# JuliaDSP/DSP.jl

Hardware: AMD Instinct MI355X
Metric: Gsamples/s filt+welch, 1 Gsample Float32 stream; achieved HBM GB/s vs roofline (higher is better)
Workload: dtype f32; 1 GPU; filt(256 taps, overlap-save nfft 2048) + welch_pgram(nfft 4096, hanning, 50 %) per 2^30-sample Float32 stream; one stream per GPU; RCCL all-reduce of the PSD for N>1; samples_per_gpu=1073741824, engine=fused, collective=none (1 GPU), collective_check=not run (--full checks it)

## Files before the change

### dsp.jl_amd/csrc/fft_lds.h

```cpp
#pragma once

#include <utility>

#ifdef __HIPCC__
#define MDSP_HD __host__ __device__ __forceinline__
#else
#define MDSP_HD inline
#endif
#if defined(__HIP_DEVICE_COMPILE__)
#define MDSP_OPAQUE_INT(x) asm volatile("" : "+v"(x))
#else
#define MDSP_OPAQUE_INT(x) (void)(x)
#endif

namespace mdsp {
namespace fft {

template <typename R> struct cx {
    R x, y;
};

template <typename R> MDSP_HD cx<R> cadd(cx<R> a, cx<R> b) { return {a.x + b.x, a.y + b.y}; }
template <typename R> MDSP_HD cx<R> csub(cx<R> a, cx<R> b) { return {a.x - b.x, a.y - b.y}; }
template <typename R> MDSP_HD cx<R> cmul(cx<R> a, cx<R> b) { return {a.x * b.x - a.y * b.y, a.x * b.y + a.y * b.x}; }
template <typename R> MDSP_HD cx<R> cmulc(cx<R> a, cx<R> b) { return {a.x * b.x + a.y * b.y, a.y * b.x - a.x * b.y}; }
template <int DIR, typename R> MDSP_HD cx<R> twmul(cx<R> a, cx<R> w) { return DIR < 0 ? cmul(a, w) : cmulc(a, w); }
template <int DIR, typename R> MDSP_HD cx<R> mul_mi(cx<R> a) { return DIR < 0 ? cx<R>{a.y, -a.x} : cx<R>{-a.y, a.x}; }

template <int DIR, typename R> MDSP_HD cx<R> add_mi(cx<R> a, cx<R> b) { return cadd(a, mul_mi<DIR>(b)); }
template <int DIR, typename R> MDSP_HD cx<R> sub_mi(cx<R> a, cx<R> b) { return csub(a, mul_mi<DIR>(b)); }
template <typename R> MDSP_HD cx<R> caxpy(R h, cx<R> u, cx<R> e) { return {e.x + h * u.x, e.y + h * u.y}; }
template <typename R> MDSP_HD cx<R> caxmy(R h, cx<R> u, cx<R> e) { return {e.x - h * u.x, e.y - h * u.y}; }
template <typename R> MDSP_HD cx<R> cscale(R h, cx<R> u) { return {h * u.x, h * u.y}; }
template <typename R> MDSP_HD cx<R> lanefma(cx<R> a, cx<R> b, cx<R> c) { return {a.x * b.x + c.x, a.y * b.y + c.y}; }
template <typename R> MDSP_HD cx<R> wmul_hi(cx<R> a, cx<R> w) { return {a.x * w.y, a.y * w.y}; }
template <typename R> MDSP_HD cx<R> wfma_lo(cx<R> a, cx<R> w, cx<R> c) { return {a.x * w.x + c.x, a.y * w.x + c.y}; }
template <typename R> MDSP_HD cx<R> wfms_lo(cx<R> a, cx<R> w, cx<R> c) { return {a.x * w.x - c.x, a.y * w.x - c.y}; }
template <int DIR, typename R> MDSP_HD cx<R> twmul_k(cx<R> a, cx<R> w) { return twmul<DIR>(a, w); }
template <typename R> MDSP_HD cx<R> cscale_k(R h, cx<R> u) { return cscale(h, u); }
template <typename R> MDSP_HD cx<R> caxpy_k(R h, cx<R> u, cx<R> e) { return caxpy(h, u, e); }
template <typename R> MDSP_HD cx<R> caxmy_k(R h, cx<R> u, cx<R> e) { return caxmy(h, u, e); }

#if defined(__HIP_DEVICE_COMPILE__) && !defined(MDSP_NO_PACKED_F32)
typedef float f2v __attribute__((ext_vector_type(2)));
#define MDSP_PK2(NAME, INSN, MODS)                                                                  \
    __device__ __forceinline__ cx<float> NAME(cx<float> a, cx<float> b) {                           \
        f2v d;                                                                                      \
        asm(INSN " %0, %1, %2 " MODS : "=v"(d) : "v"(f2v{a.x, a.y}), "v"(f2v{b.x, b.y}));           \
        return {d.x, d.y};                                                                          \
    }
#define MDSP_PK3(NAME, INSN, MODS)                                                                  \
    __device__ __forceinline__ cx<float> NAME(cx<float> a, cx<float> b, cx<float> c) {              \
        f2v d;                                                                                      \
        asm(INSN " %0, %1, %2, %3 " MODS : "=v"(d) : "v"(f2v{a.x, a.y}), "v"(f2v{b.x, b.y}), "v"(f2v{c.x, c.y})); \
        return {d.x, d.y};                                                                          \
    }
#ifndef MDSP_PK_NATIVE
#define MDSP_PK_NATIVE 0
#endif
#if MDSP_PK_NATIVE
#define MDSP_V(a) (f2v{(a).x, (a).y})
__device__ __forceinline__ cx<float> mdsp_c(f2v d) { return {d.x, d.y}; }
__device__ __forceinline__ cx<float> cadd(cx<float> a, cx<float> b) { return mdsp_c(MDSP_V(a) + MDSP_V(b)); }
__device__ __forceinline__ cx<float> csub(cx<float> a, cx<float> b) { return mdsp_c(MDSP_V(a) - MDSP_V(b)); }
#else
MDSP_PK2(cadd, "v_pk_add_f32", "")
MDSP_PK2(csub, "v_pk_add_f32", "neg_lo:[0,1] neg_hi:[0,1]")
#endif
MDSP_PK2(pk_add_ib, "v_pk_add_f32", "op_sel:[0,1] op_sel_hi:[1,0] neg_lo:[0,1]")
MDSP_PK2(pk_sub_ib, "v_pk_add_f32", "op_sel:[0,1] op_sel_hi:[1,0] neg_hi:[0,1]")
#if MDSP_PK_NATIVE
__device__ __forceinline__ cx<float> pk_mul(cx<float> a, cx<float> b) { return mdsp_c(MDSP_V(a) * MDSP_V(b)); }
__device__ __forceinline__ cx<float> pk_mul_swap(cx<float> a, cx<float> b) { return mdsp_c(f2v{a.y, a.x} * MDSP_V(b)); }
__device__ __forceinline__ cx<float> pk_mul_blo(cx<float> a, cx<float> b) { return mdsp_c(MDSP_V(a) * f2v{b.x, b.x}); }
// ... 128 lines not shown
    b = t;
}

#if defined(__HIP_DEVICE_COMPILE__) && !defined(MDSP_NO_PACKED_F32) && MDSP_PK_FUSED
template <int DIR> __device__ __forceinline__ void bfly4(cx<float>& a0, cx<float>& a1, cx<float>& a2, cx<float>& a3) {
    f2v r0 = {a0.x, a0.y}, r1 = {a1.x, a1.y}, r2 = {a2.x, a2.y}, r3 = {a3.x, a3.y}, t;
    if constexpr (DIR < 0)
        asm("v_pk_add_f32 %4, %0, %2\n\t"
            "v_pk_add_f32 %2, %0, %2 neg_lo:[0,1] neg_hi:[0,1]\n\t"
            "v_pk_add_f32 %0, %1, %3\n\t"
            "v_pk_add_f32 %3, %1, %3 neg_lo:[0,1] neg_hi:[0,1]\n\t"
            "v_pk_add_f32 %1, %4, %0 neg_lo:[0,1] neg_hi:[0,1]\n\t"
            "v_pk_add_f32 %0, %4, %0\n\t"
            "v_pk_add_f32 %4, %2, %3 op_sel:[0,1] op_sel_hi:[1,0] neg_hi:[0,1]\n\t"
            "v_pk_add_f32 %3, %2, %3 op_sel:[0,1] op_sel_hi:[1,0] neg_lo:[0,1]"
            : "+v"(r0), "+v"(r1), "+v"(r2), "+v"(r3), "=&v"(t));
    else
        asm("v_pk_add_f32 %4, %0, %2\n\t"
            "v_pk_add_f32 %2, %0, %2 neg_lo:[0,1] neg_hi:[0,1]\n\t"
            "v_pk_add_f32 %0, %1, %3\n\t"
            "v_pk_add_f32 %3, %1, %3 neg_lo:[0,1] neg_hi:[0,1]\n\t"
            "v_pk_add_f32 %1, %4, %0 neg_lo:[0,1] neg_hi:[0,1]\n\t"
            "v_pk_add_f32 %0, %4, %0\n\t"
            "v_pk_add_f32 %4, %2, %3 op_sel:[0,1] op_sel_hi:[1,0] neg_lo:[0,1]\n\t"
            "v_pk_add_f32 %3, %2, %3 op_sel:[0,1] op_sel_hi:[1,0] neg_hi:[0,1]"
            : "+v"(r0), "+v"(r1), "+v"(r2), "+v"(r3), "=&v"(t));
    a0 = {r0.x, r0.y};
    a1 = {t.x, t.y};
    a2 = {r1.x, r1.y};
    a3 = {r3.x, r3.y};
}
#endif

template <int DIR, typename R> MDSP_HD void bfly4(cx<R>& a0, cx<R>& a1, cx<R>& a2, cx<R>& a3) {
    const cx<R> t0 = cadd(a0, a2), t1 = csub(a0, a2), t2 = cadd(a1, a3), d = csub(a1, a3);
    a0 = cadd(t0, t2);
    a2 = csub(t0, t2);
    a1 = add_mi<DIR>(t1, d);
    a3 = sub_mi<DIR>(t1, d);
}

template <int DIR, typename R> MDSP_HD cx<R> w8_1_unscaled(cx<R> o) { return add_mi<DIR>(o, o); }
template <int DIR, typename R> MDSP_HD cx<R> w8_3_unscaled_neg(cx<R> o) { return sub_mi<DIR>(o, o); }

template <int DIR, typename R> MDSP_HD void bfly8(cx<R> (&v)[8]) {
    constexpr R h = (R)0.70710678118654752440084436210485L;
    bfly4<DIR>(v[0], v[2], v[4], v[6]);
    bfly4<DIR>(v[1], v[3], v[5], v[7]);
    const cx<R> e0 = v[0], e1 = v[2], e2 = v[4], e3 = v[6];
    const cx<R> o0 = v[1], o2 = v[5];
    const cx<R> u1 = w8_1_unscaled<DIR>(v[3]);
    const cx<R> u3 = w8_3_unscaled_neg<DIR>(v[7]);
    v[0] = cadd(e0, o0);
    v[4] = csub(e0, o0);
    v[1] = caxpy_k(h, u1, e1);
    v[5] = caxmy_k(h, u1, e1);
    v[2] = add_mi<DIR>(e2, o2);
    v[6] = sub_mi<DIR>(e2, o2);
    v[3] = caxmy_k(h, u3, e3);
    v[7] = caxpy_k(h, u3, e3);
}

template <int DIR, typename R> MDSP_HD void bfly16_tail(cx<R> (&v)[16]) {
    constexpr R c1 = (R)0.92387953251128675612818318939679L;
    constexpr R s1 = (R)0.38268343236508977172845998403040L;
    constexpr R h = (R)0.70710678118654752440084436210485L;
    const cx<R> w1 = {c1, -s1}, w3 = {s1, -c1}, w9 = {-c1, s1};
    v[1 + 4 * 1] = twmul_k<DIR>(v[1 + 4 * 1], w1);
    v[1 + 4 * 2] = cscale_k(h, w8_1_unscaled<DIR>(v[1 + 4 * 2]));
    v[1 + 4 * 3] = twmul_k<DIR>(v[1 + 4 * 3], w3);
    v[2 + 4 * 1] = cscale_k(h, w8_1_unscaled<DIR>(v[2 + 4 * 1]));
    v[2 + 4 * 2] = mul_mi<DIR>(v[2 + 4 * 2]);
    v[2 + 4 * 3] = cscale_k(-h, w8_3_unscaled_neg<DIR>(v[2 + 4 * 3]));
    v[3 + 4 * 1] = twmul_k<DIR>(v[3 + 4 * 1], w3);
    v[3 + 4 * 2] = cscale_k(-h, w8_3_unscaled_neg<DIR>(v[3 + 4 * 2]));
    v[3 + 4 * 3] = twmul_k<DIR>(v[3 + 4 * 3], w9);
#pragma unroll
    for (int q = 0; q < 4; ++q) bfly4<DIR>(v[4 * q + 0], v[4 * q + 1], v[4 * q + 2], v[4 * q + 3]);
    cx<R> t;
#define MDSP_SWAP(a, b) \
    t = v[a];           \
    v[a] = v[b];        \
    v[b] = t;
    MDSP_SWAP(1, 4) MDSP_SWAP(2, 8) MDSP_SWAP(3, 12) MDSP_SWAP(6, 9) MDSP_SWAP(7, 13) MDSP_SWAP(11, 14)
#undef MDSP_SWAP
}

template <int DIR, typename R> MDSP_HD void bfly16(cx<R> (&v)[16]) {
#pragma unroll
    for (int m = 0; m < 4; ++m) bfly4<DIR>(v[m], v[m + 4], v[m + 8], v[m + 12]);
    bfly16_tail<DIR>(v);
}

template <int DIR, typename R> MDSP_HD void bfly16_win(const cx<R> (&q)[8], const cx<R> (&f)[8], const cx<R> (&wp)[8], cx<R> (&v)[16]) {
#pragma unroll
    for (int m = 0; m < 4; ++m) {
        const cx<R> p0 = wmul_hi(f[m], wp[m]), p1 = wmul_hi(f[m + 4], wp[m + 4]);
        const cx<R> t0 = wfma_lo(q[m], wp[m], p0), t1 = wfms_lo(q[m], wp[m], p0);
        const cx<R> t2 = wfma_lo(q[m + 4], wp[m + 4], p1), d = wfms_lo(q[m + 4], wp[m + 4], p1);
        v[m] = cadd(t0, t2);
        v[m + 8] = csub(t0, t2);
        v[m + 4] = add_mi<DIR>(t1, d);
        v[m + 12] = sub_mi<DIR>(t1, d);
    }
    bfly16_tail<DIR>(v);
}

template <int RDX, int DIR, typename R> MDSP_HD void bfly(cx<R> (&v)[RDX]) {
    if constexpr (RDX == 2) bfly2<DIR>(v[0], v[1]);
    else if constexpr (RDX == 4) bfly4<DIR>(v[0], v[1], v[2], v[3]);
    else if constexpr (RDX == 8) bfly8<DIR>(v);
    else bfly16<DIR>(v);
}

template <int DIR, int RDX, typename R> MDSP_HD void twmul_all(cx<R> (&v)[RDX], const cx<R> (&w)[RDX]) {
#if defined(__HIP_DEVICE_COMPILE__) && !defined(MDSP_NO_PACKED_F32) && MDSP_PK_FUSED
    if constexpr (sizeof(R) == 4) {
#pragma unroll
        for (int r = 1; r + 1 < RDX; r += 2) cmul2(v[r], w[r], v[r + 1], w[r + 1], DIR > 0);
        if constexpr (((RDX - 1) & 1) != 0) v[RDX - 1] = twmul<DIR>(v[RDX - 1], w[RDX - 1]);
        return;
    }
#endif
#pragma unroll
    for (int r = 1; r < RDX; ++r) v[r] = twmul<DIR>(v[r], w[r]);
}

template <int N_, int E_> struct Cfg {
    static constexpr int N = N_, E = E_, T = N_ / E_;
    static constexpr int LOGN = ilog2(N_), LOGE = ilog2(E_);
    static_assert((1 << LOGN) == N_ && (1 << LOGE) == E_, "power of two sizes only");
    static_assert(E_ >= 2 && E_ <= 64 && N_ >= E_, "unsupported elements-per-thread");
    static constexpr int LOGR = LOGE < 4 ? LOGE : 4;
    static constexpr int P = (LOGN + LOGR - 1) / LOGR;
    static constexpr int logradix(int p) { return LOGN / P + (p < LOGN % P ? 1 : 0); }
    static constexpr int radix(int p) { return 1 << logradix(p); }
    static constexpr int ns(int p) { return p == 0 ? 1 : ns(p - 1) * radix(p - 1); }
    static constexpr int ntw(int p) { return p == 0 ? 0 : E - E / radix(p); }
    static constexpr int twoff(int p) { return p == 0 ? 0 : twoff(p - 1) + ntw(p - 1); }
    static constexpr int NTW = twoff(P - 1) + ntw(P - 1);
    static constexpr int ldstw(int p) { return p == 0 ? 0 : (radix(p) - 1) * ns(p); }
    static constexpr int ldsoff(int p) { return p <= 1 ? 0 : ldsoff(p - 1) + ldstw(p - 1); }
    static constexpr int NTWLDS = P <= 1 ? 1 : ldsoff(P - 1) + ldstw(P - 1);
};

enum { TW_GLOBAL = 0, TW_REG = 1, TW_LDS = 2, TW_HYB = 3 };
constexpr int HYB_NS_MAX = 16;
template <typename C, int TWMODE, int PASS> constexpr bool tw_pass_in_lds() {
    return TWMODE == TW_LDS || (TWMODE == TW_HYB && PASS >= 1 && C::ns(PASS) <= HYB_NS_MAX);
}
template <typename C, int TWMODE, int PASS> constexpr bool tw_pass_in_regs() {
    return TWMODE == TW_REG || (TWMODE == TW_HYB && !(PASS >= 1 && C::ns(PASS) <= HYB_NS_MAX));
}
template <typename C, int TWMODE, int PASS = 1> constexpr int tw_lds_entries() {
    if constexpr (PASS >= C::P) return 1;
    else if constexpr (tw_pass_in_lds<C, TWMODE, PASS>()) {
        constexpr int here = C::ldsoff(PASS) + C::ldstw(PASS), rest = tw_lds_entries<C, TWMODE, PASS + 1>();
        return here > rest ? here : rest;
    } else return tw_lds_entries<C, TWMODE, PASS + 1>();
// ... 10 lines not shown
        }
        fill_lds_twiddles<C, R, PASS + 1, TWMODE>(twl, t, table);
    }
}

template <int PADSHIFT> MDSP_HD int lds_pad(int i) {
    if constexpr (PADSHIFT >= 31) return i;
    else return i + (i >> PADSHIFT);
}
template <int N, int PADSHIFT> constexpr int lds_elems() { return PADSHIFT >= 31 ? N : N + (N >> PADSHIFT); }
template <int PADSHIFT> constexpr int lds_padc(int c) { return PADSHIFT >= 31 ? c : c + (c >> PADSHIFT); }

template <typename C, int PASS> MDSP_HD int tw_index(int t, int b, int r) {
    constexpr int Ns = C::ns(PASS), Rdx = C::radix(PASS);
    const int j = t + C::T * b;
    const int k = j & (Ns - 1);
    return (r * k * (C::N / (Ns * Rdx))) & (C::N - 1);
}

template <typename C, typename R, int PASS = 1, int TWMODE = TW_REG>
MDSP_HD void load_twiddles(cx<R> (&tw)[C::NTW > 0 ? C::NTW : 1], int t, const cx<R>* table) {
    if constexpr (PASS < C::P) {
        if constexpr (tw_pass_in_regs<C, TWMODE, PASS>()) {
            constexpr int Rdx = C::radix(PASS), NB = C::E / Rdx;
#pragma unroll
            for (int b = 0; b < NB; ++b)
#pragma unroll
                for (int r = 1; r < Rdx; ++r) tw[C::twoff(PASS) + b * (Rdx - 1) + (r - 1)] = table[tw_index<C, PASS>(t, b, r)];
        }
        load_twiddles<C, R, PASS + 1, TWMODE>(tw, t, table);
    }
}

template <typename C, int DIR, int PASS, int TWMODE, int PADSHIFT, typename R>
MDSP_HD void pass_compute(cx<R> (&x)[C::E], int t, const cx<R> (&tw)[C::NTW > 0 ? C::NTW : 1], const cx<R>* table, cx<R>* lds) {
    constexpr int Rdx = C::radix(PASS), NB = C::E / Rdx, Ns = C::ns(PASS);
    constexpr bool LAST = PASS == C::P - 1;
#pragma unroll
    for (int b = 0; b < NB; ++b) {
        cx<R> v[Rdx];
#pragma unroll
        for (int r = 0; r < Rdx; ++r) v[r] = x[b + r * NB];
        if constexpr (PASS > 0) {
            [[maybe_unused]] int kt = (Ns > C::T) ? t : (t & (Ns - 1));
            constexpr bool IN_LDS = tw_pass_in_lds<C, TWMODE, PASS>(), IN_REGS = tw_pass_in_regs<C, TWMODE, PASS>();
            if constexpr (IN_LDS) MDSP_OPAQUE_INT(kt);
            cx<R> wv[Rdx];
#pragma unroll
            for (int r = 1; r < Rdx; ++r) {
                if constexpr (IN_REGS) wv[r] = tw[C::twoff(PASS) + b * (Rdx - 1) + (r - 1)];
                else if constexpr (IN_LDS) {
                    const int KB = (C::T * b) & (Ns - 1);
                    wv[r] = table[kt + (C::ldsoff(PASS) + (r - 1) * Ns + KB)];
                } else wv[r] = table[tw_index<C, PASS>(t, b, r)];
            }
            twmul_all<DIR, Rdx>(v, wv);
        }
        bfly<Rdx, DIR>(v);
        if constexpr (LAST) {
#pragma unroll
            for (int r = 0; r < Rdx; ++r) x[b + r * NB] = v[r];
        } else {
            const int j = t + C::T * b;
            const int base = lds_pad<PADSHIFT>((j / Ns) * (Ns * Rdx) + (j & (Ns - 1)));
#pragma unroll
            for (int r = 0; r < Rdx; ++r) lds[base + lds_padc<PADSHIFT>(r * Ns)] = v[r];
        }
    }
}

template <typename C, int PADSHIFT, typename R> MDSP_HD void pass0_scatter(const cx<R> (&v)[16], int t, cx<R>* lds) {
    const int base = lds_pad<PADSHIFT>(t * 16);
#pragma unroll
    for (int r = 0; r < 16; ++r) lds[base + lds_padc<PADSHIFT>(r)] = v[r];
}
template <typename C, int PADSHIFT, typename R>
MDSP_HD void pass0_windowed(const cx<R> (&q)[8], const cx<R> (&f)[8], const cx<R> (&wp)[8], int t, cx<R>* lds) {
    static_assert(C::E == 16 && C::radix(0) == 16 && C::P > 1, "E = 16 geometries with a radix-16 first pass");
    cx<R> v[16];
    bfly16_win<-1>(q, f, wp, v);
    pass0_scatter<C, PADSHIFT>(v, t, lds);
}

template <typename C, int PADSHIFT, typename R> MDSP_HD void pass_reload(cx<R> (&x)[C::E], int t, const cx<R>* lds) {
    if constexpr (PADSHIFT >= 31 || C::T % (1 << (PADSHIFT >= 31 ? 0 : PADSHIFT)) == 0) {
        const int base = lds_pad<PADSHIFT>(t);
#pragma unroll
        for (int e = 0; e < C::E; ++e) x[e] = lds[base + lds_padc<PADSHIFT>(C::T * e)];
    } else {
#pragma unroll
        for (int e = 0; e < C::E; ++e) x[e] = lds[lds_pad<PADSHIFT>(t + C::T * e)];
    }
}


template <typename R> MDSP_HD void bfly3f(cx<R>& a0, cx<R>& a1, cx<R>& a2) {
    constexpr R s = (R)0.86602540378443864676372317075294L;
    const cx<R> t1 = cadd(a1, a2), d = csub(a1, a2);
    const cx<R> t2 = caxmy_k((R)0.5, t1, a0);
    const cx<R> t3 = cscale_k(s, d);
    a0 = cadd(a0, t1);
    a1 = add_mi<-1>(t2, t3);
    a2 = sub_mi<-1>(t2, t3);
}
template <typename R> MDSP_HD void bfly5f(cx<R> (&v)[5]) {
    constexpr R c1 = (R)0.30901699437494742410229341718282L, c2 = (R)-0.80901699437494742410229341718282L;
    constexpr R s1 = (R)0.95105651629515357211643933337938L, s2 = (R)0.58778525229247312916870595463907L;
    const cx<R> t1 = cadd(v[1], v[4]), t2 = cadd(v[2], v[3]), t3 = csub(v[1], v[4]), t4 = csub(v[2], v[3]);
    const cx<R> m1 = caxpy_k(c2, t2, caxpy_k(c1, t1, v[0]));
    const cx<R> m2 = caxpy_k(c1, t2, caxpy_k(c2, t1, v[0]));
    const cx<R> n1 = caxpy_k(s2, t4, cscale_k(s1, t3));
    const cx<R> n2 = caxmy_k(s1, t4, cscale_k(s2, t3));
    v[0] = cadd(v[0], cadd(t1, t2));
// ... 196 lines not shown
```

### dsp.jl_amd/csrc/fft_wg.h

```cpp
#pragma once

#include <hip/hip_runtime.h>

#include "fft_lds.h"

#ifndef MDSP_FFT_SETPRIO
#define MDSP_FFT_SETPRIO 0
#endif

namespace mdsp {
namespace fft {

template <int T> __device__ __forceinline__ void wg_sync() {
    if constexpr (T <= 64) __builtin_amdgcn_wave_barrier();
    else __syncthreads();
}

template <typename C, int PADSHIFT, int NBUF> constexpr int wg_lds_elems() { return NBUF * lds_elems<C::N, PADSHIFT>(); }

template <typename C, int DIR, int TWMODE, int PADSHIFT, int NBUF, int XBASE, int PASS = 0, typename R>
__device__ __forceinline__ void wg_fft(cx<R> (&v)[C::E], int t, const cx<R> (&tw)[C::NTW > 0 ? C::NTW : 1], const cx<R>* table, cx<R>* lds) {
    constexpr int BUF = (XBASE + PASS) % NBUF;
    cx<R>* region = lds + BUF * lds_elems<C::N, PADSHIFT>();
    pass_compute<C, DIR, PASS, TWMODE, PADSHIFT>(v, t, tw, table, region);
    if constexpr (PASS < C::P - 1) {
#if MDSP_FFT_SETPRIO
        __builtin_amdgcn_s_setprio(1);
#endif
        wg_sync<C::T>();
        pass_reload<C, PADSHIFT>(v, t, region);
        if constexpr (NBUF == 1) wg_sync<C::T>();
#if MDSP_FFT_SETPRIO
        __builtin_amdgcn_s_setprio(0);
#endif
        wg_fft<C, DIR, TWMODE, PADSHIFT, NBUF, XBASE, PASS + 1>(v, t, tw, table, lds);
    }
}

template <typename C, int TWMODE, typename R>
__device__ __forceinline__ const cx<R>* wg_twiddle_setup(cx<R> (&tw)[C::NTW > 0 ? C::NTW : 1], cx<R>* twl, int t, int slot, const cx<R>* table) {
    if constexpr (TWMODE == TW_REG) {
        load_twiddles<C, R, 1, TW_REG>(tw, t, table);
        return table;
    } else if constexpr (TWMODE == TW_LDS) {
        if (slot == 0) fill_lds_twiddles<C, R>(twl, t, table);
        __syncthreads();
        return twl;
    } else if constexpr (TWMODE == TW_HYB) {
        load_twiddles<C, R, 1, TW_HYB>(tw, t, table);
        if (slot == 0) fill_lds_twiddles<C, R, 1, TW_HYB>(twl, t, table);
        __syncthreads();
        return twl;
    } else {
        return table;
    }
}

template <typename C> constexpr int wg_exchanges() { return C::P - 1; }

}
}
```

### dsp.jl_amd/csrc/ols.hip

```cpp
#include <algorithm>
#include <atomic>
#include <cstdlib>

#ifndef MDSP_FFT_SGPR_CONST
#define MDSP_FFT_SGPR_CONST 0
#endif

#include "common.h"
#include "devio.h"
#include "fft_lds.h"
#include "fft_wg.h"
#include "hostfft.h"
#include "rocfft_wrap.h"
#include "ols_plan.h"

using namespace mdsp;
using mdsp::fft::cx;

namespace {

template <typename T>
__global__ __launch_bounds__(256) void ols_segment_kernel(const T* __restrict__ x, T* __restrict__ td, int64_t nx, int64_t ldx,
                                                          int64_t nblocks, int64_t L, int nb, int nfft, int64_t u0, int64_t nunits) {
    const int64_t u = u0 + blockIdx.x;
// ... 93 lines not shown
    {
        const __amdgpu_buffer_rsrc_t r = io::make_rsrc(xc + start, q.live ? (a.nx - start) * SZ : 0);
        const int lead = __builtin_amdgcn_readfirstlane((int)(start < 0 ? -start : 0));
        io::load_window<TT, E, T>(raw.a, r, lead, t);
    }
    if constexpr (!CPLX) {
        const bool haveB = q.live && (g0 + 1) < a.nblocks;
        const int64_t startB = start + a.L;
        const __amdgpu_buffer_rsrc_t r = io::make_rsrc(xc + startB, haveB ? (a.nx - startB) * SZ : 0);
        const int lead = __builtin_amdgcn_readfirstlane((int)(startB < 0 ? -startB : 0));
        io::load_window<TT, E, T>(raw.b, r, lead, t);
    }
}

template <typename R, int E, int T, bool CPLX>
__device__ __forceinline__ void ols_store(const cx<R> (&v)[E], const OlsFusedArgs& a, OlsPos q, int t) {
    using TT = std::conditional_t<CPLX, cx<R>, R>;
    constexpr int64_t SZ = (int64_t)sizeof(TT);
    const int64_t off0 = (CPLX ? q.p : 2 * q.p) * a.L;
    const int lead = a.nb - 1;
    TT* yc = static_cast<TT*>(a.y) + q.col * a.ldy;
    {
        const __amdgpu_buffer_rsrc_t w = io::make_rsrc(yc + off0 - lead, q.live ? (a.nout - off0 + lead) * SZ : 0);
        if constexpr (CPLX) io::store_window<TT, E, T>([&](int e) { return v[e]; }, w, lead, t);
        else io::store_window<TT, E, T>([&](int e) { return v[e].x; }, w, lead, t);
    }
    if constexpr (!CPLX) {
        const int64_t offB = off0 + a.L;
        const __amdgpu_buffer_rsrc_t w = io::make_rsrc(yc + offB - lead, (q.live && offB < a.nout) ? (a.nout - offB + lead) * SZ : 0);
        io::store_window<TT, E, T>([&](int e) { return v[e].y; }, w, lead, t);
    }
}

template <typename R, int N, int E, int G, int TWMODE, bool CPLX, int NBUF, bool PREFETCH, bool HREG = true, bool ROWS = false>
__global__ __launch_bounds__((N / E) * G, 2) void ols_fused_kernel(OlsFusedArgs a) {
    static_assert(!ROWS || (CPLX && !HREG), "the rows form: complex blocks, one spectrum row per block");
    using C = fft::Cfg<N, E>;
    constexpr int T = C::T, PADSHIFT = 4;
    static_assert(T % 64 == 0, "a transform must own whole wavefronts (uniform descriptors)");
    constexpr int NTWA = C::NTW > 0 ? C::NTW : 1;
    constexpr int REGION = fft::wg_lds_elems<C, PADSHIFT, NBUF>();
    __shared__ __attribute__((aligned(16))) cx<R> lds_all[G * REGION];
    const int t = threadIdx.x % T;
    const int slot = __builtin_amdgcn_readfirstlane((int)(threadIdx.x / T));
    cx<R>* lds = lds_all + slot * REGION;
    const cx<R>* table = static_cast<const cx<R>*>(a.table);

    cx<R> tw[NTWA];
    __shared__ __attribute__((aligned(16))) cx<R> twl[(TWMODE == fft::TW_LDS || TWMODE == fft::TW_HYB) ? fft::tw_lds_entries<C, TWMODE>() : 1];
    const cx<R>* twsrc = fft::wg_twiddle_setup<C, TWMODE>(tw, twl, t, slot, table);
    cx<R> Hr[HREG ? E : 1];
    if constexpr (HREG) {
#pragma unroll
        for (int e = 0; e < E; ++e) Hr[e] = static_cast<const cx<R>*>(a.H)[t + T * e];
    }
    const __amdgpu_buffer_rsrc_t hrsrc = io::make_rsrc(a.H, (int64_t)N * (int64_t)sizeof(cx<R>));

    const int64_t nslots = (int64_t)gridDim.x * G;
    OlsWalk walk{a.u_begin + ((int64_t)blockIdx.x * G + slot) * a.run_len, 0};
    OlsPos cur = ols_pos(a, walk, a.niter > 0);
    OlsRaw<R, E, CPLX> raw;
    if constexpr (PREFETCH) ols_issue_loads<R, E, T, CPLX>(raw, a, cur, t);
    for (int64_t it = 0; it < a.niter; ++it) {
        ols_walk_next(walk, a.run_len, nslots);
        const OlsPos nxt = ols_pos(a, walk, it + 1 < a.niter);
        if constexpr (!PREFETCH) {
            if (!MDSP_ABLATED(a, 1)) {
                if (a.memprio & 1) __builtin_amdgcn_s_setprio(3);
                ols_issue_loads<R, E, T, CPLX>(raw, a, cur, t);
                if (a.memprio & 1) __builtin_amdgcn_s_setprio(0);
            }
        }
        cx<R> v[E];
#pragma unroll
        for (int e = 0; e < E; ++e) {
            if constexpr (CPLX) v[e] = raw.a[e];
            else v[e] = {raw.a[e], raw.b[e]};
        }
        if constexpr (PREFETCH) { if (!MDSP_ABLATED(a, 1)) ols_issue_loads<R, E, T, CPLX>(raw, a, nxt, t); }
        if (!MDSP_ABLATED(a, 2)) {
        fft::wg_fft<C, -1, TWMODE, PADSHIFT, NBUF, 0>(v, t, tw, twsrc, lds);
        if constexpr (HREG) {
#pragma unroll
            for (int e = 0; e < E; ++e) v[e] = fft::cmul(v[e], Hr[e]);
        } else {
            cx<R> hh[E];
            if constexpr (ROWS) {
                const __amdgpu_buffer_rsrc_t hrow = io::make_rsrc(static_cast<const cx<R>*>(a.H) + (cur.p % a.hrows) * N, (int64_t)N * (int64_t)sizeof(cx<R>));
                io::load_window<cx<R>, E, T>(hh, hrow, 0, t);
            } else
            io::load_window<cx<R>, E, T>(hh, hrsrc, 0, t);
#pragma unroll
            for (int e = 0; e < E; ++e) v[e] = fft::cmul(v[e], hh[e]);
        }
        fft::wg_fft<C, +1, TWMODE, PADSHIFT, NBUF, (C::P - 1) % NBUF>(v, t, tw, twsrc, lds);
        if constexpr (ROWS) {
            const cx<R>*t0 = static_cast<const cx<R>*>(a.rt0), *t1 = static_cast<const cx<R>*>(a.rt1);
            const unsigned k1 = (unsigned)(cur.p % a.hrows), mask = (1u << a.rlogS) - 1u;
            const auto root = [&](unsigned m) { return fft::cmul(t0[m & mask], t1[m >> a.rlogS]); };
            const cx<R> w0 = root(k1 * (unsigned)t);
#pragma unroll
            for (int e = 0; e < E; ++e) {
                const cx<R> w = fft::cmul(w0, root(k1 * (unsigned)(T * e)));
                v[e] = fft::cmul(v[e], cx<R>{w.x, -w.y});
            }
        }
        }
        if (!MDSP_ABLATED(a, 4)) {
            if (a.memprio & 2) __builtin_amdgcn_s_setprio(3);
            ols_store<R, E, T, CPLX>(v, a, cur, t);
            if (a.memprio & 2) __builtin_amdgcn_s_setprio(0);
        }
        cur = nxt;
    }
}

struct UpolsArgs {
    const void* x;
    void* y;
    const void* table;
    const void* Hp;
    int64_t nx, nout, ldx, ldy;
    int64_t nblocks;
    int64_t g_begin;
    int64_t x_lo;
    int64_t run_len;
    int ablate;
    int memprio;
// ... 365 lines not shown
        return true;
    }
    for (int64_t n = 4096; n <= nmax; n *= 2) {
        const int64_t parts = cdiv(nb, n / 2);
        if (parts <= 4) {
            *exec_nfft = n;
            *partitions = (int)std::max<int64_t>(2, parts);
            return true;
        }
    }
    return false;
}

template <typename R> int upload_spectrum(mdsp_ols_plan_s* pl, const std::vector<zd>& Hfull, bool half) {
    const int64_t n = half ? pl->nfft / 2 + 1 : pl->nfft;
    std::vector<cx<R>> h((size_t)n);
    for (int64_t k = 0; k < n; ++k) h[(size_t)k] = {(R)Hfull[(size_t)k].real(), (R)Hfull[(size_t)k].imag()};
    MDSP_TRY(pl->H.reserve(sizeof(cx<R>) * (size_t)n));
    MDSP_HIP(hipMemcpy(pl->H.p, h.data(), sizeof(cx<R>) * (size_t)n, hipMemcpyHostToDevice));
    return MDSP_OK;
}

template <typename R> int upload_table(DevBuf& buf, int64_t n) {
    std::vector<cx<R>> w((size_t)n);
    for (int64_t k = 0; k < n; ++k) {
        const zd r = unit_root(k, n, -1);
        w[(size_t)k] = {(R)r.real(), (R)r.imag()};
    }
    MDSP_TRY(buf.reserve(sizeof(cx<R>) * (size_t)n));
    MDSP_HIP(hipMemcpy(buf.p, w.data(), sizeof(cx<R>) * (size_t)n, hipMemcpyHostToDevice));
    return MDSP_OK;
}

template <typename R, int N, int E, int G, int TWMODE, bool CPLX, int NBUF, bool PREFETCH, bool HREG = true, bool ROWS = false>
int launch_fused_geo(const OlsFusedArgs& a, hipStream_t s) {
    auto kern = ols_fused_kernel<R, N, E, G, TWMODE, CPLX, NBUF, PREFETCH, HREG, ROWS>;
    constexpr int threads = (N / E) * G;
    int per_cu = 0;
    MDSP_HIP(hipOccupancyMaxActiveBlocksPerMultiprocessor(&per_cu, kern, threads, 0));
    if (per_cu < 1) per_cu = 1;
    if (tunables().wg_per_cu > 0) per_cu = tunables().wg_per_cu;
    const int64_t todo = a.nunits - a.u_begin;
    const int64_t want = cdiv(todo, G);
    const int grid = (int)std::max<int64_t>(1, std::min<int64_t>(want, (int64_t)device_cu_count() * per_cu));
    OlsFusedArgs b = a;
    const int64_t runs = tunables().runs_per_slot;
    const int64_t nslots = (int64_t)grid * G;
    b.run_len = std::max<int64_t>(1, cdiv(todo, nslots * runs));
    b.niter = cdiv(cdiv(todo, b.run_len), nslots) * b.run_len;
    hipLaunchKernelGGL(kern, dim3(grid), dim3(threads), 0, s, b);
    MDSP_LAUNCH_CHECK();
    return MDSP_OK;
}

int ols_rows_impl(int dbl, void* work, int64_t rows, int hrows, const void* Hrows, const void* table, const void* rt0, const void* rt1, int rlogS, hipStream_t st) {
    OlsFusedArgs a{};
    const int64_t S = dbl ? 4096 : 8192;
    a.x = work;
    a.y = work;
    a.table = table;
    a.H = Hrows;
    a.nx = a.nout = a.ldx = a.ldy = rows * S;
    a.L = S;
    a.nb = 1;
    a.nblocks = a.units_per_col = a.nunits = rows;
    a.u_begin = 0;
    a.memprio = tunables().ols_prio;
    a.hrows = hrows;
    a.rt0 = rt0;
    a.rt1 = rt1;
    a.rlogS = rlogS;
    if (dbl) return launch_fused_geo<double, 4096, 8, 1, 1, true, 2, false, false, true>(a, st);
    return launch_fused_geo<float, 8192, 16, 1, 1, true, 1, false, false, true>(a, st);
}

template <typename R, int N, bool CPLX> int launch_fused_n(const OlsFusedArgs& a, hipStream_t s) {
    constexpr bool DBL = sizeof(R) == 8;
    constexpr int EMAX = (!DBL && N >= 1024) ? 16 : 8;
    constexpr int E = (N / 64 < EMAX) ? N / 64 : EMAX;
    constexpr int T = N / E;
    constexpr int G = slots_per_workgroup(T);
    constexpr int NBUF = (T <= 64 || E == 16) ? 1 : 2;
#ifndef MDSP_TW_F64
#define MDSP_TW_F64 1
#endif
    constexpr int TWREG = DBL ? MDSP_TW_F64 : 1;
    if constexpr (N == 2048 && !CPLX && !DBL) return launch_fused_geo<R, N, 16, 1, 1, CPLX, 1, false>(a, s);
    if (tunables().ols_prefetch == 1) return launch_fused_geo<R, N, E, G, TWREG, CPLX, NBUF, true>(a, s);
    return launch_fused_geo<R, N, E, G, TWREG, CPLX, NBUF, false>(a, s);
}

template <typename R, bool CPLX> int launch_fused(int64_t nfft, const OlsFusedArgs& a, hipStream_t s) {
    switch (nfft) {
        case 256: return launch_fused_n<R, 256, CPLX>(a, s);
        case 512: return launch_fused_n<R, 512, CPLX>(a, s);
        case 1024: return launch_fused_n<R, 1024, CPLX>(a, s);
        case 2048: return launch_fused_n<R, 2048, CPLX>(a, s);
        case 4096: return launch_fused_n<R, 4096, CPLX>(a, s);
        case 8192:
            if constexpr (sizeof(R) == 4) return launch_fused_n<R, 8192, CPLX>(a, s);
        default: break;
    }
    MDSP_FAIL(MDSP_ERR_UNSUPPORTED, "fused overlap-save does not support nfft=%lld", (long long)nfft);
}

struct UpolsRange {
    int64_t g0, g1, x_lo;
};
template <typename R, int N, int E, int P, bool CPLX, int MINW, bool XDMA, int NLDS = 0, int FORM = 1, bool H0REG = false>
int launch_upols_k(const mdsp_ols_plan_s* pl, const void* x, int64_t nx, int64_t ncols, int64_t ldx, void* y, int64_t nout, int64_t ldy, UpolsRange rg, hipStream_t s) {
    constexpr bool DBL = sizeof(R) == 8;
    constexpr int TW = DBL ? 1 : fft::TW_HYB;
    void (*kern)(UpolsArgs) = nullptr;
    if constexpr (FORM == 2) kern = upols2_fused_kernel<R, N, E, P, TW, 4, CPLX, MINW, NLDS, H0REG>;
    else kern = upols_fused_kernel<R, N, E, P, TW, 4, CPLX, MINW, XDMA, NLDS>;
    constexpr int threads = N / E, RUNS = CPLX ? 1 : 2;
    UpolsArgs a;
    a.x = x; a.y = y; a.table = pl->table.p; a.Hp = pl->H.p;
    a.nx = nx; a.nout = nout; a.ldx = ldx; a.ldy = ldy;
    a.nblocks = rg.g1;
    a.g_begin = rg.g0;
    a.x_lo = rg.x_lo;
// ... 422 lines not shown
```

Baseline: 366.8 Gsamples/s.

## Fold twiddle multiplies into radix-16/8 butterflies and fuse spectrum multiply into inverse FFT

Adds folded butterfly variants that merge each twiddle multiply into the first butterfly stage with FMA (including packed-f32 inline-asm versions). For the real nfft=2048 overlap-save path it also folds the filter spectrum multiply into the first radix-16 pass of the inverse FFT, and uses folded twiddle passes for later stages. The aim is fewer VALU instructions per FFT in a kernel that may be compute-bound. In exchange it adds a large amount of hand-written asm with intricate modifier encodings, which risks numerical or sign errors and could raise register pressure.

```diff
diff --git a/dsp.jl_amd/csrc/fft_lds.h b/dsp.jl_amd/csrc/fft_lds.h
--- a/dsp.jl_amd/csrc/fft_lds.h
+++ b/dsp.jl_amd/csrc/fft_lds.h
@@ -40,6 +40,22 @@
 template <typename R> MDSP_HD cx<R> cscale_k(R h, cx<R> u) { return cscale(h, u); }
 template <typename R> MDSP_HD cx<R> caxpy_k(R h, cx<R> u, cx<R> e) { return caxpy(h, u, e); }
 template <typename R> MDSP_HD cx<R> caxmy_k(R h, cx<R> u, cx<R> e) { return caxmy(h, u, e); }
+
+MDSP_HD float fma1(float a, float b, float c) { return __builtin_fmaf(a, b, c); }
+MDSP_HD double fma1(double a, double b, double c) { return __builtin_fma(a, b, c); }
+template <typename R> struct cx2 {
+    cx<R> plus, minus;
+};
+template <int DIR, typename R> MDSP_HD cx2<R> fold(cx<R> a, cx<R> b, cx<R> w) {
+    const R wy = DIR < 0 ? w.y : -w.y;
+    const cx<R> t = {fma1(b.y, -wy, a.x), fma1(b.y, w.x, a.y)};
+    const cx<R> p = {fma1(b.x, w.x, t.x), fma1(b.x, wy, t.y)};
+    return {p, {fma1(a.x, (R)2, -p.x), fma1(a.y, (R)2, -p.y)}};
+}
+template <int DIR, typename R> MDSP_HD cx2<R> fold_mi(cx<R> a, cx<R> b) { return {add_mi<DIR>(a, b), sub_mi<DIR>(a, b)}; }
+template <typename R> MDSP_HD cx2<R> fold_re(cx<R> a, R h, cx<R> u) {
+    return {{fma1(u.x, h, a.x), fma1(u.y, h, a.y)}, {fma1(-u.x, h, a.x), fma1(-u.y, h, a.y)}};
+}
 
 #if defined(__HIP_DEVICE_COMPILE__) && !defined(MDSP_NO_PACKED_F32)
 typedef float f2v __attribute__((ext_vector_type(2)));
@@ -234,6 +250,90 @@
 }
 #endif
 
+#if defined(__HIP_DEVICE_COMPILE__) && !defined(MDSP_NO_PACKED_F32) && MDSP_PK_FUSED
+#define MDSP_M_SUB " neg_lo:[0,1] neg_hi:[0,1]"
+#define MDSP_M_ADD_IB " op_sel:[0,1] op_sel_hi:[1,0] neg_lo:[0,1]"
+#define MDSP_M_SUB_IB " op_sel:[0,1] op_sel_hi:[1,0] neg_hi:[0,1]"
+#define MDSP_M_YY " op_sel:[1,1] op_sel_hi:[1,0]"
+#define MDSP_M_FIN_F " op_sel_hi:[0,1,1] neg_lo:[0,0,1]"
+#define MDSP_M_FIN_I " op_sel_hi:[0,1,1] neg_hi:[1,0,0]"
+#define MDSP_M_FA_F " op_sel:[1,1,0] op_sel_hi:[1,0,1] neg_lo:[0,1,0]"
+#define MDSP_M_FA_I " op_sel:[1,1,0] op_sel_hi:[1,0,1]"
+#define MDSP_M_FB_F " op_sel_hi:[0,1,1]"
+#define MDSP_M_FB_I " op_sel_hi:[0,1,1] neg_hi:[0,1,0]"
+#define MDSP_M_F2 " op_sel_hi:[1,0,1] neg_lo:[0,0,1] neg_hi:[0,0,1]"
+#define MDSP_M_NEGA " neg_lo:[1,0,0] neg_hi:[1,0,0]"
+#define MDSP_BFLY4_TW(FA, FB, X1, X3)                                                                                         \
+    asm("v_pk_fma_f32 %4, %2, %6, %0" FA "\n\tv_pk_fma_f32 %5, %3, %7, %1" FA "\n\t"                                            \
+        "v_pk_fma_f32 %4, %2, %6, %4" FB "\n\tv_pk_fma_f32 %5, %3, %7, %5" FB "\n\t"                      \
+        "v_pk_fma_f32 %2, %0, 2.0, %4" MDSP_M_F2 "\n\tv_pk_fma_f32 %3, %1, 2.0, %5" MDSP_M_F2 "\n\t"        \
+        "v_pk_add_f32 %0, %4, %5\n\tv_pk_add_f32 %1, %4, %5" MDSP_M_SUB "\n\t"                                                  \
+        "v_pk_add_f32 %4, %2, %3" X1 "\n\tv_pk_add_f32 %3, %2, %3" X3                                                           \
+        : "+v"(r0), "+v"(r1), "+v"(r2), "+v"(r3), "=&v"(t), "=&v"(u) : "v"(f2v{w2.x, w2.y}), "v"(f2v{w3.x, w3.y}))
+template <int DIR, int WDIR> __device__ __forceinline__ void bfly4_tw(cx<float>& a0, cx<float>& a1, cx<float>& a2, cx<float>& a3, cx<float> w2, cx<float> w3) {
+    f2v r0 = {a0.x, a0.y}, r1 = {a1.x, a1.y}, r2 = {a2.x, a2.y}, r3 = {a3.x, a3.y}, t, u;
+    if constexpr (DIR < 0 && WDIR < 0) MDSP_BFLY4_TW(MDSP_M_FA_F, MDSP_M_FB_F, MDSP_M_SUB_IB, MDSP_M_ADD_IB);
+    else if constexpr (DIR < 0) MDSP_BFLY4_TW(MDSP_M_FA_I, MDSP_M_FB_I, MDSP_M_SUB_IB, MDSP_M_ADD_IB);
+    else if constexpr (WDIR < 0) MDSP_BFLY4_TW(MDSP_M_FA_F, MDSP_M_FB_F, MDSP_M_ADD_IB, MDSP_M_SUB_IB);
+    else MDSP_BFLY4_TW(MDSP_M_FA_I, MDSP_M_FB_I, MDSP_M_ADD_IB, MDSP_M_SUB_IB);
+    a0 = {r0.x, r0.y};
+    a1 = {t.x, t.y};
+    a2 = {r1.x, r1.y};
+    a3 = {r3.x, r3.y};
+}
+#undef MDSP_BFLY4_TW
+#define MDSP_BFLY4_W16_13(FIN, UMOD, T0NEG, T1NEG, FA, FB, X1, X3)                                                              \
+    asm("v_pk_mul_f32 %4, %1, %6" MDSP_M_YY "\n\tv_pk_add_f32 %5, %2, %2" UMOD "\n\t"                                             \
+        "v_pk_fma_f32 %4, %1, %6, %4" FIN "\n\t"                                                              \
+        "v_pk_fma_f32 %1, %5, %7, %0" T0NEG "\n\tv_pk_fma_f32 %2, %5, %7, %0" T1NEG "\n\t"                  \
+        "v_pk_fma_f32 %5, %3, %8, %4" FA "\n\tv_pk_fma_f32 %5, %3, %8, %5" FB "\n\t"                                 \
+        "v_pk_fma_f32 %3, %4, 2.0, %5" MDSP_M_F2 "\n\t"                                                              \
+        "v_pk_add_f32 %0, %1, %5\n\tv_pk_add_f32 %4, %1, %5" MDSP_M_SUB "\n\t"                                                    \
+        "v_pk_add_f32 %1, %2, %3" X1 "\n\tv_pk_add_f32 %3, %2, %3" X3                                                             \
+        : "+v"(r0), "+v"(r1), "+v"(r2), "+v"(r3), "=&v"(t), "=&v"(u) : "v"(f2v{wa.x, wa.y}), "v"(f2v{h, h}), "v"(f2v{wb.x, wb.y}))
+#define MDSP_BFLY4_W16_2(MI_ADD, MI_SUB)                                                                                         \
+    asm("v_pk_add_f32 %4, %1, %1" MI_ADD "\n\tv_pk_add_f32 %5, %3, %3" MI_SUB "\n\t"                                              \
+        "v_pk_mul_f32 %4, %4, %6\n\t"                                                                            \
+        "v_pk_add_f32 %1, %0, %2" MI_ADD "\n\tv_pk_add_f32 %2, %0, %2" MI_SUB "\n\t"                        \
+        "v_pk_fma_f32 %0, %5, %6, %4" MDSP_M_NEGA "\n\tv_pk_fma_f32 %3, %5, %6, %4\n\t"                      \
+        "v_pk_add_f32 %5, %1, %0\n\tv_pk_add_f32 %4, %1, %0" MDSP_M_SUB "\n\t"                                                    \
+        "v_pk_add_f32 %1, %2, %3" MI_ADD "\n\tv_pk_add_f32 %3, %2, %3" MI_SUB                                                     \
+        : "+v"(r0), "+v"(r1), "+v"(r2), "+v"(r3), "=&v"(t), "=&v"(u) : "v"(f2v{h, h}))
+template <int DIR, int Q> __device__ __forceinline__ void bfly4_w16(cx<float>& a0, cx<float>& a1, cx<float>& a2, cx<float>& a3) {
+    constexpr float c1 = 0.92387953251128675612818318939679f, s1 = 0.38268343236508977172845998403040f, h = 0.70710678118654752440084436210485f;
+    constexpr cx<float> wa = Q == 1 ? cx<float>{c1, -s1} : cx<float>{s1, -c1}, wb = Q == 1 ? cx<float>{s1, -c1} : cx<float>{-c1, s1};
+    f2v r0 = {a0.x, a0.y}, r1 = {a1.x, a1.y}, r2 = {a2.x, a2.y}, r3 = {a3.x, a3.y}, t, u;
+    if constexpr (Q == 2) {
+        if constexpr (DIR < 0) MDSP_BFLY4_W16_2(MDSP_M_SUB_IB, MDSP_M_ADD_IB);
+        else MDSP_BFLY4_W16_2(MDSP_M_ADD_IB, MDSP_M_SUB_IB);
+        a0 = {u.x, u.y};
+    } else {
+        if constexpr (Q == 1 && DIR < 0) MDSP_BFLY4_W16_13(MDSP_M_FIN_F, MDSP_M_SUB_IB, "", MDSP_M_NEGA, MDSP_M_FA_F, MDSP_M_FB_F, MDSP_M_SUB_IB, MDSP_M_ADD_IB);
+        else if constexpr (Q == 1) MDSP_BFLY4_W16_13(MDSP_M_FIN_I, MDSP_M_ADD_IB, "", MDSP_M_NEGA, MDSP_M_FA_I, MDSP_M_FB_I, MDSP_M_ADD_IB, MDSP_M_SUB_IB);
+        else if constexpr (DIR < 0) MDSP_BFLY4_W16_13(MDSP_M_FIN_F, MDSP_M_ADD_IB, MDSP_M_NEGA, "", MDSP_M_FA_F, MDSP_M_FB_F, MDSP_M_SUB_IB, MDSP_M_ADD_IB);
+        else MDSP_BFLY4_W16_13(MDSP_M_FIN_I, MDSP_M_SUB_IB, MDSP_M_NEGA, "", MDSP_M_FA_I, MDSP_M_FB_I, MDSP_M_ADD_IB, MDSP_M_SUB_IB);
+        a0 = {r0.x, r0.y};
+    }
+    a1 = {r1.x, r1.y};
+    a2 = {t.x, t.y};
+    a3 = {r3.x, r3.y};
+}
+#undef MDSP_BFLY4_W16_13
+#undef MDSP_BFLY4_W16_2
+#undef MDSP_M_SUB
+#undef MDSP_M_ADD_IB
+#undef MDSP_M_SUB_IB
+#undef MDSP_M_YY
+#undef MDSP_M_FIN_F
+#undef MDSP_M_FIN_I
+#undef MDSP_M_FA_F
+#undef MDSP_M_FA_I
+#undef MDSP_M_FB_F
+#undef MDSP_M_FB_I
+#undef MDSP_M_F2
+#undef MDSP_M_NEGA
+#endif
+
 template <int DIR, typename R> MDSP_HD void bfly4(cx<R>& a0, cx<R>& a1, cx<R>& a2, cx<R>& a3) {
     const cx<R> t0 = cadd(a0, a2), t1 = csub(a0, a2), t2 = cadd(a1, a3), d = csub(a1, a3);
     a0 = cadd(t0, t2);
@@ -245,10 +345,8 @@
 template <int DIR, typename R> MDSP_HD cx<R> w8_1_unscaled(cx<R> o) { return add_mi<DIR>(o, o); }
 template <int DIR, typename R> MDSP_HD cx<R> w8_3_unscaled_neg(cx<R> o) { return sub_mi<DIR>(o, o); }
 
-template <int DIR, typename R> MDSP_HD void bfly8(cx<R> (&v)[8]) {
+template <int DIR, typename R> MDSP_HD void bfly8_tail(cx<R> (&v)[8]) {
     constexpr R h = (R)0.70710678118654752440084436210485L;
-    bfly4<DIR>(v[0], v[2], v[4], v[6]);
-    bfly4<DIR>(v[1], v[3], v[5], v[7]);
     const cx<R> e0 = v[0], e1 = v[2], e2 = v[4], e3 = v[6];
     const cx<R> o0 = v[1], o2 = v[5];
     const cx<R> u1 = w8_1_unscaled<DIR>(v[3]);
@@ -262,8 +360,49 @@
     v[3] = caxmy_k(h, u3, e3);
     v[7] = caxpy_k(h, u3, e3);
 }
-
-template <int DIR, typename R> MDSP_HD void bfly16_tail(cx<R> (&v)[16]) {
+template <int DIR, typename R> MDSP_HD void bfly8(cx<R> (&v)[8]) {
+    bfly4<DIR>(v[0], v[2], v[4], v[6]);
+    bfly4<DIR>(v[1], v[3], v[5], v[7]);
+    bfly8_tail<DIR>(v);
+}
+
+template <int DIR, int WDIR, typename R> MDSP_HD void bfly4_tw(cx<R>& a0, cx<R>& a1, cx<R>& a2, cx<R>& a3, cx<R> w2, cx<R> w3) {
+    const cx2<R> e = fold<WDIR>(a0, a2, w2), o = fold<WDIR>(a1, a3, w3);
+    a0 = cadd(e.plus, o.plus);
+    a2 = csub(e.plus, o.plus);
+    a1 = add_mi<DIR>(e.minus, o.minus);
+    a3 = sub_mi<DIR>(e.minus, o.minus);
+}
+template <int DIR, int Q, typename R> MDSP_HD void bfly4_w16(cx<R>& a0, cx<R>& a1, cx<R>& a2, cx<R>& a3) {
+    constexpr R c1 = (R)0.92387953251128675612818318939679L, s1 = (R)0.38268343236508977172845998403040L, h = (R)0.70710678118654752440084436210485L;
+    const cx<R> w1 = {c1, -s1}, w3 = {s1, -c1}, w9 = {-c1, s1};
+    cx2<R> e, o;
+    if constexpr (Q == 1) {
+        const cx<R> p = twmul_k<DIR>(a1, w1);
+        e = fold_re(a0, h, w8_1_unscaled<DIR>(a2));
+        o = fold<DIR>(p, a3, w3);
+    } else if constexpr (Q == 2) {
+        const cx<R> p = cscale_k(h, w8_1_unscaled<DIR>(a1));
+        e = fold_mi<DIR>(a0, a2);
+        o = fold_re(p, -h, w8_3_unscaled_neg<DIR>(a3));
+    } else {
+        const cx<R> p = twmul_k<DIR>(a1, w3);
+        e = fold_re(a0, -h, w8_3_unscaled_neg<DIR>(a2));
+        o = fold<DIR>(p, a3, w9);
+    }
+    a0 = cadd(e.plus, o.plus);
+    a2 = csub(e.plus, o.plus);
+    a1 = add_mi<DIR>(e.minus, o.minus);
+    a3 = sub_mi<DIR>(e.minus, o.minus);
+}
+
+template <int DIR, bool FOLD = false, typename R> MDSP_HD void bfly16_tail(cx<R> (&v)[16]) {
+    if constexpr (FOLD) {
+        bfly4<DIR>(v[0], v[1], v[2], v[3]);
+        bfly4_w16<DIR, 1>(v[4], v[5], v[6], v[7]);
+        bfly4_w16<DIR, 2>(v[8], v[9], v[10], v[11]);
+        bfly4_w16<DIR, 3>(v[12], v[13], v[14], v[15]);
+    } else {
     constexpr R c1 = (R)0.92387953251128675612818318939679L;
     constexpr R s1 = (R)0.38268343236508977172845998403040L;
     constexpr R h = (R)0.70710678118654752440084436210485L;
@@ -279,6 +418,7 @@
     v[3 + 4 * 3] = twmul_k<DIR>(v[3 + 4 * 3], w9);
 #pragma unroll
     for (int q = 0; q < 4; ++q) bfly4<DIR>(v[4 * q + 0], v[4 * q + 1], v[4 * q + 2], v[4 * q + 3]);
+    }
     cx<R> t;
 #define MDSP_SWAP(a, b) \
     t = v[a];           \
@@ -288,10 +428,10 @@
 #undef MDSP_SWAP
 }
 
-template <int DIR, typename R> MDSP_HD void bfly16(cx<R> (&v)[16]) {
+template <int DIR, bool FOLD = false, typename R> MDSP_HD void bfly16(cx<R> (&v)[16]) {
 #pragma unroll
     for (int m = 0; m < 4; ++m) bfly4<DIR>(v[m], v[m + 4], v[m + 8], v[m + 12]);
-    bfly16_tail<DIR>(v);
+    bfly16_tail<DIR, FOLD>(v);
 }
 
 template <int DIR, typename R> MDSP_HD void bfly16_win(const cx<R> (&q)[8], const cx<R> (&f)[8], const cx<R> (&wp)[8], cx<R> (&v)[16]) {
@@ -327,6 +467,33 @@
 #pragma unroll
     for (int r = 1; r < RDX; ++r) v[r] = twmul<DIR>(v[r], w[r]);
 }
+
+template <int WDIR, int RDX, bool W0, typename R> MDSP_HD void twmul_first(cx<R> (&v)[RDX], const cx<R> (&w)[RDX]) {
+    constexpr int HALF = RDX / 2, R0 = W0 ? 0 : 1;
+#if defined(__HIP_DEVICE_COMPILE__) && !defined(MDSP_NO_PACKED_F32) && MDSP_PK_FUSED
+    if constexpr (sizeof(R) == 4) {
+#pragma unroll
+        for (int r = R0; r + 1 < HALF; r += 2) cmul2(v[r], w[r], v[r + 1], w[r + 1], WDIR > 0);
+        if constexpr (((HALF - R0) & 1) != 0) v[HALF - 1] = twmul<WDIR>(v[HALF - 1], w[HALF - 1]);
+        return;
+    }
+#endif
+#pragma unroll
+    for (int r = R0; r < HALF; ++r) v[r] = twmul<WDIR>(v[r], w[r]);
+}
+template <int DIR, int WDIR = DIR, bool W0 = false, typename R> MDSP_HD void bfly16_tw(cx<R> (&v)[16], const cx<R> (&w)[16]) {
+    twmul_first<WDIR, 16, W0>(v, w);
+#pragma unroll
+    for (int m = 0; m < 4; ++m) bfly4_tw<DIR, WDIR>(v[m], v[m + 4], v[m + 8], v[m + 12], w[m + 8], w[m + 12]);
+    bfly16_tail<DIR, true>(v);
+}
+template <int DIR, typename R> MDSP_HD void bfly8_tw(cx<R> (&v)[8], const cx<R> (&w)[8]) {
+    twmul_first<DIR, 8, false>(v, w);
+    bfly4_tw<DIR, DIR>(v[0], v[2], v[4], v[6], w[4], w[6]);
+    bfly4_tw<DIR, DIR>(v[1], v[3], v[5], v[7], w[5], w[7]);
+    bfly8_tail<DIR>(v);
+}
+template <int DIR, typename R> MDSP_HD void bfly16_h(cx<R> (&v)[16], const cx<R> (&H)[16]) { bfly16_tw<DIR, -1, true>(v, H); }
 
 template <int N_, int E_> struct Cfg {
     static constexpr int N = N_, E = E_, T = N_ / E_;
@@ -403,10 +570,11 @@
     }
 }
 
-template <typename C, int DIR, int PASS, int TWMODE, int PADSHIFT, typename R>
+template <typename C, int DIR, int PASS, int TWMODE, int PADSHIFT, bool FOLD = false, typename R>
 MDSP_HD void pass_compute(cx<R> (&x)[C::E], int t, const cx<R> (&tw)[C::NTW > 0 ? C::NTW : 1], const cx<R>* table, cx<R>* lds) {
     constexpr int Rdx = C::radix(PASS), NB = C::E / Rdx, Ns = C::ns(PASS);
     constexpr bool LAST = PASS == C::P - 1;
+    constexpr bool FOLDED_TW = FOLD && PASS > 0 && (Rdx == 16 || Rdx == 8);
 #pragma unroll
     for (int b = 0; b < NB; ++b) {
         cx<R> v[Rdx];
@@ -425,9 +593,14 @@
                     wv[r] = table[kt + (C::ldsoff(PASS) + (r - 1) * Ns + KB)];
                 } else wv[r] = table[tw_index<C, PASS>(t, b, r)];
             }
-            twmul_all<DIR, Rdx>(v, wv);
+            if constexpr (FOLDED_TW && Rdx == 16) bfly16_tw<DIR>(v, wv);
+            else if constexpr (FOLDED_TW) bfly8_tw<DIR>(v, wv);
+            else twmul_all<DIR, Rdx>(v, wv);
         }
-        bfly<Rdx, DIR>(v);
+        if constexpr (!FOLDED_TW) {
+            if constexpr (FOLD && Rdx == 16) bfly16<DIR, true>(v);
+            else bfly<Rdx, DIR>(v);
+        }
         if constexpr (LAST) {
 #pragma unroll
             for (int r = 0; r < Rdx; ++r) x[b + r * NB] = v[r];
@@ -450,6 +623,12 @@
     static_assert(C::E == 16 && C::radix(0) == 16 && C::P > 1, "E = 16 geometries with a radix-16 first pass");
     cx<R> v[16];
     bfly16_win<-1>(q, f, wp, v);
+    pass0_scatter<C, PADSHIFT>(v, t, lds);
+}
+
+template <typename C, int DIR, int PADSHIFT, typename R> MDSP_HD void pass0_spectrum(cx<R> (&v)[16], const cx<R> (&H)[16], int t, cx<R>* lds) {
+    static_assert(C::E == 16 && C::radix(0) == 16 && C::P > 1, "E = 16 geometries with a radix-16 first pass");
+    bfly16_h<DIR>(v, H);
     pass0_scatter<C, PADSHIFT>(v, t, lds);
 }
 
diff --git a/dsp.jl_amd/csrc/fft_wg.h b/dsp.jl_amd/csrc/fft_wg.h
--- a/dsp.jl_amd/csrc/fft_wg.h
+++ b/dsp.jl_amd/csrc/fft_wg.h
@@ -18,11 +18,11 @@
 
 template <typename C, int PADSHIFT, int NBUF> constexpr int wg_lds_elems() { return NBUF * lds_elems<C::N, PADSHIFT>(); }
 
-template <typename C, int DIR, int TWMODE, int PADSHIFT, int NBUF, int XBASE, int PASS = 0, typename R>
+template <typename C, int DIR, int TWMODE, int PADSHIFT, int NBUF, int XBASE, int PASS = 0, bool FOLD = false, typename R>
 __device__ __forceinline__ void wg_fft(cx<R> (&v)[C::E], int t, const cx<R> (&tw)[C::NTW > 0 ? C::NTW : 1], const cx<R>* table, cx<R>* lds) {
     constexpr int BUF = (XBASE + PASS) % NBUF;
     cx<R>* region = lds + BUF * lds_elems<C::N, PADSHIFT>();
-    pass_compute<C, DIR, PASS, TWMODE, PADSHIFT>(v, t, tw, table, region);
+    pass_compute<C, DIR, PASS, TWMODE, PADSHIFT, FOLD>(v, t, tw, table, region);
     if constexpr (PASS < C::P - 1) {
 #if MDSP_FFT_SETPRIO
         __builtin_amdgcn_s_setprio(1);
@@ -33,8 +33,17 @@
 #if MDSP_FFT_SETPRIO
         __builtin_amdgcn_s_setprio(0);
 #endif
-        wg_fft<C, DIR, TWMODE, PADSHIFT, NBUF, XBASE, PASS + 1>(v, t, tw, table, lds);
+        wg_fft<C, DIR, TWMODE, PADSHIFT, NBUF, XBASE, PASS + 1, FOLD>(v, t, tw, table, lds);
     }
+}
+
+template <typename C, int DIR, int TWMODE, int PADSHIFT, typename R>
+__device__ __forceinline__ void wg_fft_spectrum(cx<R> (&v)[C::E], const cx<R> (&H)[C::E], int t, const cx<R> (&tw)[C::NTW > 0 ? C::NTW : 1], const cx<R>* table, cx<R>* lds) {
+    pass0_spectrum<C, DIR, PADSHIFT>(v, H, t, lds);
+    wg_sync<C::T>();
+    pass_reload<C, PADSHIFT>(v, t, lds);
+    wg_sync<C::T>();
+    wg_fft<C, DIR, TWMODE, PADSHIFT, 1, 0, 1, true>(v, t, tw, table, lds);
 }
 
 template <typename C, int TWMODE, typename R>
diff --git a/dsp.jl_amd/csrc/ols.hip b/dsp.jl_amd/csrc/ols.hip
--- a/dsp.jl_amd/csrc/ols.hip
+++ b/dsp.jl_amd/csrc/ols.hip
@@ -149,9 +149,10 @@
     }
 }
 
-template <typename R, int N, int E, int G, int TWMODE, bool CPLX, int NBUF, bool PREFETCH, bool HREG = true, bool ROWS = false>
+template <typename R, int N, int E, int G, int TWMODE, bool CPLX, int NBUF, bool PREFETCH, bool HREG = true, bool ROWS = false, bool FOLD = false>
 __global__ __launch_bounds__((N / E) * G, 2) void ols_fused_kernel(OlsFusedArgs a) {
     static_assert(!ROWS || (CPLX && !HREG), "the rows form: complex blocks, one spectrum row per block");
+    static_assert(!FOLD || (HREG && NBUF == 1 && E == 16), "the folded form: spectrum in registers, one LDS buffer");
     using C = fft::Cfg<N, E>;
     constexpr int T = C::T, PADSHIFT = 4;
     static_assert(T % 64 == 0, "a transform must own whole wavefronts (uniform descriptors)");
@@ -196,7 +197,10 @@
         }
         if constexpr (PREFETCH) { if (!MDSP_ABLATED(a, 1)) ols_issue_loads<R, E, T, CPLX>(raw, a, nxt, t); }
         if (!MDSP_ABLATED(a, 2)) {
-        fft::wg_fft<C, -1, TWMODE, PADSHIFT, NBUF, 0>(v, t, tw, twsrc, lds);
+        fft::wg_fft<C, -1, TWMODE, PADSHIFT, NBUF, 0, 0, FOLD>(v, t, tw, twsrc, lds);
+        if constexpr (FOLD) {
+            fft::wg_fft_spectrum<C, +1, TWMODE, PADSHIFT>(v, Hr, t, tw, twsrc, lds);
+        } else {
         if constexpr (HREG) {
 #pragma unroll
             for (int e = 0; e < E; ++e) v[e] = fft::cmul(v[e], Hr[e]);
@@ -211,6 +215,7 @@
             for (int e = 0; e < E; ++e) v[e] = fft::cmul(v[e], hh[e]);
         }
         fft::wg_fft<C, +1, TWMODE, PADSHIFT, NBUF, (C::P - 1) % NBUF>(v, t, tw, twsrc, lds);
+        }
         if constexpr (ROWS) {
             const cx<R>*t0 = static_cast<const cx<R>*>(a.rt0), *t1 = static_cast<const cx<R>*>(a.rt1);
             const unsigned k1 = (unsigned)(cur.p % a.hrows), mask = (1u << a.rlogS) - 1u;
@@ -642,9 +647,9 @@
     return MDSP_OK;
 }
 
-template <typename R, int N, int E, int G, int TWMODE, bool CPLX, int NBUF, bool PREFETCH, bool HREG = true, bool ROWS = false>
+template <typename R, int N, int E, int G, int TWMODE, bool CPLX, int NBUF, bool PREFETCH, bool HREG = true, bool ROWS = false, bool FOLD = false>
 int launch_fused_geo(const OlsFusedArgs& a, hipStream_t s) {
-    auto kern = ols_fused_kernel<R, N, E, G, TWMODE, CPLX, NBUF, PREFETCH, HREG, ROWS>;
+    auto kern = ols_fused_kernel<R, N, E, G, TWMODE, CPLX, NBUF, PREFETCH, HREG, ROWS, FOLD>;
     constexpr int threads = (N / E) * G;
     int per_cu = 0;
     MDSP_HIP(hipOccupancyMaxActiveBlocksPerMultiprocessor(&per_cu, kern, threads, 0));
@@ -695,9 +700,11 @@
 #define MDSP_TW_F64 1
 #endif
     constexpr int TWREG = DBL ? MDSP_TW_F64 : 1;
-    if constexpr (N == 2048 && !CPLX && !DBL) return launch_fused_geo<R, N, 16, 1, 1, CPLX, 1, false>(a, s);
+    if constexpr (N == 2048 && !CPLX && !DBL) return launch_fused_geo<R, N, 16, 1, 1, CPLX, 1, false, true, false, true>(a, s);
+    else {
     if (tunables().ols_prefetch == 1) return launch_fused_geo<R, N, E, G, TWREG, CPLX, NBUF, true>(a, s);
     return launch_fused_geo<R, N, E, G, TWREG, CPLX, NBUF, false>(a, s);
+    }
 }
 
 template <typename R, bool CPLX> int launch_fused(int64_t nfft, const OlsFusedArgs& a, hipStream_t s) {
```

Result: faster. 370.6 Gsamples/s, median of 6 (+1.0%).
